# vainaviv/hulk-keypoints

Measured on NVIDIA B200. Metric: heatmap_inference_images_per_sec, higher is better.
Workload: dtype bf16

## Files before the change

### hulk_keypoints_b200/csrc/conv_tc.cu

```cuda
#include <cuda.h>

#include "hk_common.cuh"
#include "hk_ptx.cuh"

namespace hk {

constexpr int TC_BLOCK_M = 128;
constexpr int TC_BLOCK_K = 64;
constexpr int TC_UMMA_K = 16;
constexpr int TC_BOX_H = 4, TC_BOX_W = 16;
constexpr int TC_BOX_PIX = TC_BOX_H * TC_BOX_W;
constexpr int TC_BOX_BYTES = TC_BOX_PIX * TC_BLOCK_K * 2;
constexpr int TC_A_BYTES = TC_BLOCK_M * TC_BLOCK_K * 2;
constexpr int TC_THREADS = 256;
constexpr int TC_EPI_WARP0 = 4;

struct ConvTcArgs {
  const float* scale;
  const float* bias;
  const __nv_bfloat16* residual;
  __nv_bfloat16* y;
  int B, Ho, Wo, Cout;
  int Cin, kh, kw, stride, pad, dil, relu;
  int tiles_x, tiles_per_img, num_boxes;
  int num_m_tiles, num_n_tiles, cblocks;
};

template <int BLOCK_N>
struct TcCfg {
  static constexpr int B_BYTES = BLOCK_N * TC_BLOCK_K * 2;
  static constexpr int STAGE_BYTES = TC_A_BYTES + B_BYTES;
  static constexpr int STAGES = (192 * 1024) / STAGE_BYTES > 8 ? 8 : (192 * 1024) / STAGE_BYTES;
  static constexpr int TMEM_COLS = 2 * BLOCK_N;
  static constexpr int SMEM_BYTES = STAGES * STAGE_BYTES + 1024  + 256 ;
};

__device__ __forceinline__ void tc_decode_box(const ConvTcArgs& a, int box, int& b, int& y0, int& x0) {
  if (box < a.num_boxes) {
    b = box / a.tiles_per_img;
    const int r = box - b * a.tiles_per_img;
    const int ty = r / a.tiles_x;
    y0 = ty * TC_BOX_H;
    x0 = (r - ty * a.tiles_x) * TC_BOX_W;
  } else {
    b = a.B;
    y0 = 0;
    x0 = 0;
  }
}

template <int BLOCK_N>
__global__ void __launch_bounds__(TC_THREADS, 1)
conv_tc_kernel(const __grid_constant__ CUtensorMap map_x, const __grid_constant__ CUtensorMap map_w, const ConvTcArgs a) {
  using Cfg = TcCfg<BLOCK_N>;
  constexpr int STAGES = Cfg::STAGES;
  extern __shared__ uint8_t smem_raw[];
  uint8_t* smem = smem_raw + ((1024u - (ptx::smem_u32(smem_raw) & 1023u)) & 1023u);
  uint64_t* full_bar = reinterpret_cast<uint64_t*>(smem + STAGES * Cfg::STAGE_BYTES);
  uint64_t* empty_bar = full_bar + STAGES;
  uint64_t* tmem_full_bar = empty_bar + STAGES;
  uint64_t* tmem_empty_bar = tmem_full_bar + 2;
  uint32_t* tmem_ptr_smem = reinterpret_cast<uint32_t*>(tmem_empty_bar + 2);

  const int warp = __shfl_sync(0xffffffffu, threadIdx.x >> 5, 0), lane = threadIdx.x & 31;
  const int total_tiles = a.num_m_tiles * a.num_n_tiles;
  const int num_kb = a.kh * a.kw * a.cblocks;

  if (warp == 0 && lane == 0) {
    ptx::prefetch_tensormap(&map_x);
    ptx::prefetch_tensormap(&map_w);
  }
  if (warp == 1 && lane == 0) {
    for (int i = 0; i < STAGES; ++i) {
      ptx::mbar_init(&full_bar[i], 1);
      ptx::mbar_init(&empty_bar[i], 1);
    }
    for (int i = 0; i < 2; ++i) {
      ptx::mbar_init(&tmem_full_bar[i], 1);
      ptx::mbar_init(&tmem_empty_bar[i], 128);
    }
    ptx::fence_mbar_init();
  }
  if (warp == 2) {
    ptx::tmem_alloc(tmem_ptr_smem, Cfg::TMEM_COLS);
    ptx::tmem_relinquish();
  }
  ptx::tc_fence_before();
  __syncthreads();
  ptx::tc_fence_after();
  const uint32_t tmem_base = *tmem_ptr_smem;

  if (warp == 0) {
    {
      uint32_t stage = 0, phase = 0;
      for (int tile = blockIdx.x; tile < total_tiles; tile += gridDim.x) {
        const int m_tile = tile / a.num_n_tiles, n_tile = tile - m_tile * a.num_n_tiles;
        int b0, y0, x0, b1, y1, x1;
        tc_decode_box(a, 2 * m_tile, b0, y0, x0);
        tc_decode_box(a, 2 * m_tile + 1, b1, y1, x1);
        for (int r = 0; r < a.kh; ++r) {
          for (int s = 0; s < a.kw; ++s) {
            const int dy = r * a.dil - a.pad, dx = s * a.dil - a.pad;
            const int kbase = (r * a.kw + s) * a.Cin;
            for (int cb = 0; cb < a.cblocks; ++cb) {
              ptx::mbar_wait(&empty_bar[stage], phase ^ 1, 1);
              if (ptx::elect_one_sync()) {
                uint8_t* sa = smem + stage * Cfg::STAGE_BYTES;
                ptx::mbar_arrive_expect_tx(&full_bar[stage], Cfg::STAGE_BYTES);
                ptx::tma_load_4d(sa, &map_x, &full_bar[stage], cb * TC_BLOCK_K, x0 * a.stride + dx, y0 * a.stride + dy, b0);
                ptx::tma_load_4d(sa + TC_BOX_BYTES, &map_x, &full_bar[stage], cb * TC_BLOCK_K, x1 * a.stride + dx,
                                 y1 * a.stride + dy, b1);
                ptx::tma_load_2d(sa + TC_A_BYTES, &map_w, &full_bar[stage], kbase + cb * TC_BLOCK_K, n_tile * BLOCK_N);
              }
              __syncwarp();
              if (++stage == STAGES) { stage = 0; phase ^= 1; }
            }
          }
        }
      }
    }
  } else if (warp == 1) {
    {
      constexpr uint32_t idesc = ptx::make_idesc_bf16_f32(TC_BLOCK_M, BLOCK_N);
      uint32_t stage = 0, phase = 0, it = 0;
      for (int tile = blockIdx.x; tile < total_tiles; tile += gridDim.x, ++it) {
        const uint32_t acc = it & 1, acc_phase = (it >> 1) & 1;
        ptx::mbar_wait(&tmem_empty_bar[acc], acc_phase ^ 1, 2);
        ptx::tc_fence_after();
        const uint32_t d_tmem = tmem_base + acc * BLOCK_N;
        for (int kb = 0; kb < num_kb; ++kb) {
          ptx::mbar_wait(&full_bar[stage], phase, 3);
          ptx::tc_fence_after();
          const uint32_t sa = ptx::smem_u32(smem + stage * Cfg::STAGE_BYTES);
          const uint64_t adesc = ptx::make_smem_desc_sw128(sa);
          const uint64_t bdesc = ptx::make_smem_desc_sw128(sa + TC_A_BYTES);
          if (ptx::elect_one_sync()) {
#pragma unroll
            for (int k = 0; k < TC_BLOCK_K / TC_UMMA_K; ++k) {
              ptx::umma_bf16(d_tmem, adesc + 2 * k, bdesc + 2 * k, idesc, (kb | k) != 0 ? 1u : 0u);
            }
            ptx::umma_commit(&empty_bar[stage]);
            if (kb == num_kb - 1) ptx::umma_commit(&tmem_full_bar[acc]);
          }
          __syncwarp();
          if (++stage == STAGES) { stage = 0; phase ^= 1; }
        }
      }
    }
  } else if (warp >= TC_EPI_WARP0) {
    const int q = warp & 3;
    const int row = q * 32 + lane;
    const int py = (row & 63) >> 4, px = row & 15;
    uint32_t it = 0;
    for (int tile = blockIdx.x; tile < total_tiles; tile += gridDim.x, ++it) {
      const uint32_t acc = it & 1, acc_phase = (it >> 1) & 1;
      const int m_tile = tile / a.num_n_tiles, n_tile = tile - m_tile * a.num_n_tiles;
      int b, y0, x0;
      tc_decode_box(a, 2 * m_tile + (row >> 6), b, y0, x0);
      const int oy = y0 + py, ox = x0 + px;
      const bool valid = (b < a.B) && (oy < a.Ho) && (ox < a.Wo);
      const size_t off = valid ? (((size_t)b * a.Ho + oy) * a.Wo + ox) * a.Cout + (size_t)n_tile * BLOCK_N : 0;
      const float* scale = a.scale + n_tile * BLOCK_N;
      const float* bias = a.bias + n_tile * BLOCK_N;

      ptx::mbar_wait(&tmem_full_bar[acc], acc_phase, 4);
      ptx::tc_fence_after();
      const uint32_t taddr = tmem_base + (static_cast<uint32_t>(q * 32) << 16) + acc * BLOCK_N;
#pragma unroll 1
      for (int c0 = 0; c0 < BLOCK_N; c0 += 32) {
        uint32_t r[32];
        ptx::tmem_ld_32x32(taddr + c0, r);
        ptx::tmem_ld_wait();
        if (valid) {
#pragma unroll
          for (int g = 0; g < 4; ++g) {
            const int c = c0 + g * 8;
            const float4 s0 = __ldg(reinterpret_cast<const float4*>(scale + c));
            const float4 s1 = __ldg(reinterpret_cast<const float4*>(scale + c + 4));
            const float4 t0 = __ldg(reinterpret_cast<const float4*>(bias + c));
            const float4 t1 = __ldg(reinterpret_cast<const float4*>(bias + c + 4));
            float v[8];
            v[0] = fmaf(__uint_as_float(r[g * 8 + 0]), s0.x, t0.x);
            v[1] = fmaf(__uint_as_float(r[g * 8 + 1]), s0.y, t0.y);
            v[2] = fmaf(__uint_as_float(r[g * 8 + 2]), s0.z, t0.z);
            v[3] = fmaf(__uint_as_float(r[g * 8 + 3]), s0.w, t0.w);
            v[4] = fmaf(__uint_as_float(r[g * 8 + 4]), s1.x, t1.x);
            v[5] = fmaf(__uint_as_float(r[g * 8 + 5]), s1.y, t1.y);
            v[6] = fmaf(__uint_as_float(r[g * 8 + 6]), s1.z, t1.z);
            v[7] = fmaf(__uint_as_float(r[g * 8 + 7]), s1.w, t1.w);
            if (a.residual) {
              const uint4 rq = __ldg(reinterpret_cast<const uint4*>(a.residual + off + c));
              float lo, hi;
              unpack_bf16x2(rq.x, lo, hi); v[0] += lo; v[1] += hi;
              unpack_bf16x2(rq.y, lo, hi); v[2] += lo; v[3] += hi;
              unpack_bf16x2(rq.z, lo, hi); v[4] += lo; v[5] += hi;
              unpack_bf16x2(rq.w, lo, hi); v[6] += lo; v[7] += hi;
            }
            if (a.relu) {
#pragma unroll
              for (int j = 0; j < 8; ++j) v[j] = fmaxf(v[j], 0.f);
            }
            *reinterpret_cast<uint4*>(a.y + off + c) =
                make_uint4(pack_bf16x2(v[0], v[1]), pack_bf16x2(v[2], v[3]), pack_bf16x2(v[4], v[5]), pack_bf16x2(v[6], v[7]));
          }
        }
      }
      ptx::tc_fence_before();
      ptx::mbar_arrive(&tmem_empty_bar[acc]);
    }
  }

  ptx::tc_fence_before();
  __syncthreads();
  if (warp == 2) {
    ptx::tc_fence_after();
    ptx::tmem_dealloc(tmem_base, Cfg::TMEM_COLS);
  }
}

typedef CUresult (*EncodeTiledFn)(CUtensorMap*, CUtensorMapDataType, cuuint32_t, void*, const cuuint64_t*, const cuuint64_t*,
                                  const cuuint32_t*, const cuuint32_t*, CUtensorMapInterleave, CUtensorMapSwizzle,
                                  CUtensorMapL2promotion, CUtensorMapFloatOOBfill);

EncodeTiledFn get_encode_fn() {
  static EncodeTiledFn fn = nullptr;
  static bool tried = false;
  if (!tried) {
    tried = true;
    void* p = nullptr;
    cudaDriverEntryPointQueryResult q;
    if (cudaGetDriverEntryPoint("cuTensorMapEncodeTiled", &p, cudaEnableDefault, &q) == cudaSuccess &&
        q == cudaDriverEntryPointSuccess)
      fn = reinterpret_cast<EncodeTiledFn>(p);
  }
  return fn;
}

template <int BLOCK_N>
static int launch_tc(const CUtensorMap& mx, const CUtensorMap& mw, const ConvTcArgs& a, cudaStream_t s) {
  using Cfg = TcCfg<BLOCK_N>;
  static bool attr_set = false;
  int dev = 0;
  cudaGetDevice(&dev);
  static int attr_dev_mask = 0;
  if (!attr_set || !(attr_dev_mask & (1 << dev))) {
    cudaError_t e = cudaFuncSetAttribute(conv_tc_kernel<BLOCK_N>, cudaFuncAttributeMaxDynamicSharedMemorySize, Cfg::SMEM_BYTES);
    if (e != cudaSuccess) return fail(HK_ERR_CUDA, "conv(tcgen05): smem attribute (%d B): %s", Cfg::SMEM_BYTES, cudaGetErrorString(e));
    attr_set = true;
    attr_dev_mask |= (1 << dev);
  }
  const int total = a.num_m_tiles * a.num_n_tiles;
  int grid = sm_count();
  if (grid > total) grid = total;
  conv_tc_kernel<BLOCK_N><<<grid, TC_THREADS, Cfg::SMEM_BYTES, s>>>(mx, mw, a);
  return check_launch("conv_tc_kernel");
}

bool conv_tc2_applicable(const HkConvDesc& d);
int conv_tc2_launch(const HkConvDesc& d, const void* x, const void* w, const float* scale, const float* bias,
                    const void* residual, void* y, void* bn_acc, cudaStream_t s);
bool conv_tc2h_applicable(const HkConvDesc& d);
int conv_tc2h_launch(const HkConvDesc& d, const void* x, const void* w, const float* scale, const float* bias,
                     const void* residual, void* y, void* bn_acc, cudaStream_t s);
bool conv_tc_c64_applicable(const HkConvDesc& d);
int conv_tc_c64_launch(const HkConvDesc& d, const void* x, const void* w, const float* scale, const float* bias,
                       const void* residual, void* y, void* bn_acc, cudaStream_t s);

int conv_tc_launch(const HkConvDesc& d, const void* x, const void* w, const float* scale, const float* bias,
                   const void* residual, void* y, cudaStream_t s, void* bn_acc = nullptr, bool* stats_done = nullptr) {
  if (stats_done) *stats_done = false;
  HK_REQUIRE(d.in_dtype == HK_BF16 && d.out_dtype == HK_BF16 && !d.in_is_nchw, "conv(tcgen05): needs NHWC bf16 in and out");
  HK_REQUIRE(d.in_c % TC_BLOCK_K == 0, "conv(tcgen05): in_c=%d must be a multiple of 64", d.in_c);
  HK_REQUIRE(d.out_c % 64 == 0, "conv(tcgen05): out_c=%d must be a multiple of 64", d.out_c);
  HK_REQUIRE(d.stride == 1 || d.stride == 2, "conv(tcgen05): stride must be 1 or 2");
  HK_REQUIRE((reinterpret_cast<uintptr_t>(x) & 15) == 0 && (reinterpret_cast<uintptr_t>(w) & 15) == 0 &&
                 (reinterpret_cast<uintptr_t>(y) & 15) == 0 && (reinterpret_cast<uintptr_t>(residual) & 15) == 0,
             "conv(tcgen05): buffers must be 16-byte aligned");
  EncodeTiledFn encode = get_encode_fn();
  if (!encode) return fail(HK_ERR_CUDA, "conv(tcgen05): cuTensorMapEncodeTiled entry point not available");

  const bool specialised = d.algo != HK_CONV_TCGEN05_1CTA;
  if (stats_done) *stats_done = bn_acc && specialised && (conv_tc_c64_applicable(d) || conv_tc2_applicable(d));
  if (specialised && conv_tc_c64_applicable(d)) return conv_tc_c64_launch(d, x, w, scale, bias, residual, y, bn_acc, s);
  if (specialised && conv_tc2_applicable(d) && conv_tc2h_applicable(d)) return conv_tc2h_launch(d, x, w, scale, bias, residual, y, bn_acc, s);
  if (specialised && conv_tc2_applicable(d)) return conv_tc2_launch(d, x, w, scale, bias, residual, y, bn_acc, s);

  const int block_n = d.out_c % 256 == 0 ? 256 : (d.out_c % 128 == 0 ? 128 : 64);
  const int ktot = d.kh * d.kw * d.in_c;

  CUtensorMap mx, mw;
  {
    const cuuint64_t dims[4] = {(cuuint64_t)d.in_c, (cuuint64_t)d.in_w, (cuuint64_t)d.in_h, (cuuint64_t)d.batch};
    const cuuint64_t strides[3] = {(cuuint64_t)d.in_c * 2, (cuuint64_t)d.in_w * d.in_c * 2, (cuuint64_t)d.in_h * d.in_w * d.in_c * 2};
    const cuuint32_t box[4] = {(cuuint32_t)TC_BLOCK_K, (cuuint32_t)(TC_BOX_W * d.stride), (cuuint32_t)(TC_BOX_H * d.stride), 1};
    const cuuint32_t estr[4] = {1, (cuuint32_t)d.stride, (cuuint32_t)d.stride, 1};
    CUresult r = encode(&mx, CU_TENSOR_MAP_DATA_TYPE_BFLOAT16, 4, const_cast<void*>(x), dims, strides, box, estr,
                        CU_TENSOR_MAP_INTERLEAVE_NONE, CU_TENSOR_MAP_SWIZZLE_128B, CU_TENSOR_MAP_L2_PROMOTION_L2_128B,
                        CU_TENSOR_MAP_FLOAT_OOB_FILL_NONE);
    if (r != CUDA_SUCCESS) return fail(HK_ERR_CUDA, "conv(tcgen05): cuTensorMapEncodeTiled(activations) failed with CUresult %d", (int)r);
  }
  {
    const cuuint64_t dims[2] = {(cuuint64_t)ktot, (cuuint64_t)d.out_c};
    const cuuint64_t strides[1] = {(cuuint64_t)ktot * 2};
    const cuuint32_t box[2] = {(cuuint32_t)TC_BLOCK_K, (cuuint32_t)block_n};
    const cuuint32_t estr[2] = {1, 1};
    CUresult r = encode(&mw, CU_TENSOR_MAP_DATA_TYPE_BFLOAT16, 2, const_cast<void*>(w), dims, strides, box, estr,
                        CU_TENSOR_MAP_INTERLEAVE_NONE, CU_TENSOR_MAP_SWIZZLE_128B, CU_TENSOR_MAP_L2_PROMOTION_L2_256B,
                        CU_TENSOR_MAP_FLOAT_OOB_FILL_NONE);
    if (r != CUDA_SUCCESS) return fail(HK_ERR_CUDA, "conv(tcgen05): cuTensorMapEncodeTiled(weights) failed with CUresult %d", (int)r);
  }

  ConvTcArgs a;
  a.scale = scale; a.bias = bias;
  a.residual = static_cast<const __nv_bfloat16*>(residual);
  a.y = static_cast<__nv_bfloat16*>(y);
  a.B = d.batch; a.Ho = d.out_h; a.Wo = d.out_w; a.Cout = d.out_c;
  a.Cin = d.in_c; a.kh = d.kh; a.kw = d.kw; a.stride = d.stride; a.pad = d.pad; a.dil = d.dil; a.relu = d.relu;
  a.tiles_x = ceil_div(d.out_w, TC_BOX_W);
  a.tiles_per_img = a.tiles_x * ceil_div(d.out_h, TC_BOX_H);
  const long long boxes = (long long)a.tiles_per_img * d.batch;
  HK_REQUIRE(boxes < 0x3fffffffLL, "conv(tcgen05): too many tiles");
  a.num_boxes = (int)boxes;
  a.num_m_tiles = (a.num_boxes + 1) / 2;
  a.num_n_tiles = d.out_c / block_n;
  a.cblocks = d.in_c / TC_BLOCK_K;
  switch (block_n) {
    case 256: return launch_tc<256>(mx, mw, a, s);
    case 128: return launch_tc<128>(mx, mw, a, s);
    default: return launch_tc<64>(mx, mw, a, s);
  }
}

int conv_ffma_launch(const HkConvDesc& d, const void* x, const void* w, const float* scale, const float* bias,
                     const void* residual, void* y, cudaStream_t s);

}

extern "C" int hk_conv_bn_act_fwd(const HkConvDesc* desc, const void* x, const void* w_packed, const float* scale,
                                  const float* bias, const void* residual_or_null, void* y, void* stream) {
  using namespace hk;
  HK_REQUIRE(desc && x && w_packed && scale && bias && y, "hk_conv_bn_act_fwd: null pointer");
  const HkConvDesc& d = *desc;
  HK_REQUIRE(d.batch > 0 && d.in_h > 0 && d.in_w > 0 && d.in_c > 0 && d.out_c > 0 && d.kh > 0 && d.kw > 0 && d.stride > 0 &&
                 d.dil > 0 && d.pad >= 0,
             "hk_conv_bn_act_fwd: bad descriptor");
  const int eh = d.dil * (d.kh - 1) + 1, ew = d.dil * (d.kw - 1) + 1;
  HK_REQUIRE(d.in_h + 2 * d.pad >= eh && d.in_w + 2 * d.pad >= ew, "hk_conv_bn_act_fwd: kernel larger than padded input");
  HK_REQUIRE(d.out_h == (d.in_h + 2 * d.pad - eh) / d.stride + 1 && d.out_w == (d.in_w + 2 * d.pad - ew) / d.stride + 1,
             "hk_conv_bn_act_fwd: out_h/out_w (%d,%d) inconsistent with the descriptor", d.out_h, d.out_w);
  if (d.algo == HK_CONV_TCGEN05 || d.algo == HK_CONV_TCGEN05_1CTA) return conv_tc_launch(d, x, w_packed, scale, bias, residual_or_null, y, as_stream(stream));
  if (d.algo == HK_CONV_FFMA) return conv_ffma_launch(d, x, w_packed, scale, bias, residual_or_null, y, as_stream(stream));
  return fail(HK_ERR_BAD_ARG, "hk_conv_bn_act_fwd: unknown algo %d", d.algo);
}

extern "C" int hk_bn_stats_acc(const void* y, long long P, int C, void* acc, void* stream);
extern "C" int hk_conv_bn_stats_fwd(const HkConvDesc* desc, const void* x, const void* w_packed, const float* scale, const float* bias,
                                    void* y, void* acc, void* stream) {
  using namespace hk;
  HK_REQUIRE(desc && x && w_packed && scale && bias && y && acc, "hk_conv_bn_stats_fwd: null pointer");
  const HkConvDesc& d = *desc;
  HK_REQUIRE(d.algo == HK_CONV_TCGEN05 && d.in_dtype == HK_BF16 && d.out_dtype == HK_BF16 && !d.in_is_nchw && !d.relu,
             "hk_conv_bn_stats_fwd: tcgen05 path only (NHWC bf16 in and out, no ReLU: BatchNorm sees the raw conv output)");
  HK_REQUIRE(d.batch > 0 && d.in_h > 0 && d.in_w > 0 && d.in_c > 0 && d.out_c > 0 && d.kh > 0 && d.kw > 0 && d.stride > 0 && d.dil > 0 && d.pad >= 0,
             "hk_conv_bn_stats_fwd: bad descriptor");
  const int eh = d.dil * (d.kh - 1) + 1, ew = d.dil * (d.kw - 1) + 1;
  HK_REQUIRE(d.out_h == (d.in_h + 2 * d.pad - eh) / d.stride + 1 && d.out_w == (d.in_w + 2 * d.pad - ew) / d.stride + 1,
             "hk_conv_bn_stats_fwd: out_h/out_w (%d,%d) inconsistent with the descriptor", d.out_h, d.out_w);
  HK_REQUIRE((reinterpret_cast<uintptr_t>(acc) & 31) == 0, "hk_conv_bn_stats_fwd: accumulators must be 32-byte aligned");
  bool done = false;
  int rc = conv_tc_launch(d, x, w_packed, scale, bias, nullptr, y, as_stream(stream), acc, &done);
  if (rc || done) return rc;
  return hk_bn_stats_acc(y, (long long)d.batch * d.out_h * d.out_w, d.out_c, acc, stream);
}
```

### hulk_keypoints_b200/csrc/conv_tc2h.cu

```cuda
#include <cuda.h>
#include <stdlib.h>

#include "hk_common.cuh"
#include "hk_bn_acc.cuh"
#include "hk_ptx.cuh"
#include "hk_ptx2.cuh"

namespace hk {

constexpr int TH_TILE_H = 8, TH_TILE_W = 16;
constexpr int TH_ROW_BYTES = TH_TILE_W * 128;
constexpr int TH_THREADS = 384;
constexpr int TH_EPI_THREADS = 256;
constexpr int TH_STAGING_BYTES = 3 * 128 * 128;
constexpr int TH_MAX_A = 4, TH_MAX_B = 8;

struct ConvTc2hArgs {
  const float* scale;
  const float* bias;
  const __nv_bfloat16* residual;
  int B, Ho, Wo, Cout, Cin, pad, dil, relu;
  int tiles_x, tiles_per_img, num_patches;
  int strip_first, num_strips, strips_per_img, strip_y0;
  int num_m_tiles, num_n_tiles, cblocks;
  int a_slot_bytes, a_bytes_full, a_bytes_strip, a_slots, b_slots;
  BnAcc* bn_acc;
};

__device__ __forceinline__ void th_decode_patch(const ConvTc2hArgs& a, int patch, int& b, int& y0, int& x0) {
  if (patch < a.num_patches) {
    b = patch / a.tiles_per_img;
    const int r = patch - b * a.tiles_per_img;
    const int ty = r / a.tiles_x;
    y0 = ty * TH_TILE_H;
    x0 = (r - ty * a.tiles_x) * TH_TILE_W;
  } else if (patch >= a.strip_first && patch < a.strip_first + a.num_strips) {
    const int q = patch - a.strip_first;
    b = q / a.strips_per_img;
    y0 = a.strip_y0;
    x0 = (q - b * a.strips_per_img) * (2 * TH_TILE_W);
  } else {
    b = a.B;
    y0 = 0;
    x0 = 0;
  }
}

template <int BLOCK_N, bool STATS>
__global__ void __cluster_dims__(2, 1, 1) __launch_bounds__(TH_THREADS, 1)
conv_tc2h_kernel(const __grid_constant__ CUtensorMap map_x, const __grid_constant__ CUtensorMap map_w,
                 const __grid_constant__ CUtensorMap map_y, const __grid_constant__ CUtensorMap map_res,
                 const __grid_constant__ CUtensorMap map_xs, const __grid_constant__ CUtensorMap map_ys,
                 const __grid_constant__ CUtensorMap map_ress, const ConvTc2hArgs a) {
  constexpr int HALF_N = BLOCK_N / 2;
  constexpr int B_BYTES = HALF_N * 128;
  extern __shared__ uint8_t smem_raw[];
  uint8_t* smem = smem_raw + ((1024u - (ptx::smem_u32(smem_raw) & 1023u)) & 1023u);
  const int NA = a.a_slots, NB = a.b_slots;
  uint8_t* sA = smem;
  uint8_t* sB = sA + NA * a.a_slot_bytes;
  uint8_t* staging = sB + NB * B_BYTES;
  uint64_t* a_full = reinterpret_cast<uint64_t*>(staging + TH_STAGING_BYTES);
  uint64_t* a_empty = a_full + TH_MAX_A;
  uint64_t* b_full = a_empty + TH_MAX_A;
  uint64_t* b_empty = b_full + TH_MAX_B;
  uint64_t* tmem_full_bar = b_empty + TH_MAX_B;
  uint64_t* tmem_empty_bar = tmem_full_bar + 2;
  uint64_t* res_bar = tmem_empty_bar + 2;
  uint32_t* tmem_ptr_smem = reinterpret_cast<uint32_t*>(res_bar + 3);

  const int warp = __shfl_sync(0xffffffffu, threadIdx.x >> 5, 0), lane = threadIdx.x & 31;
  const uint32_t rank = ptx::cluster_ctarank();
  const bool leader = rank == 0;
  const int cluster_id = blockIdx.x >> 1, num_clusters = gridDim.x >> 1;
  const int total_tiles = a.num_m_tiles * a.num_n_tiles;

  ptx::griddep_launch_dependents();
  ptx::cluster_sync_all();
  if (warp == 0 && lane == 0) {
    ptx::prefetch_tensormap(&map_x);
    ptx::prefetch_tensormap(&map_w);
    ptx::prefetch_tensormap(&map_y);
    if (a.residual) ptx::prefetch_tensormap(&map_res);
    if (a.num_strips > 0) {
      ptx::prefetch_tensormap(&map_xs);
      ptx::prefetch_tensormap(&map_ys);
      if (a.residual) ptx::prefetch_tensormap(&map_ress);
    }
  }
  if (warp == 1 && lane == 0) {
    for (int i = 0; i < TH_MAX_A; ++i) {
      ptx::mbar_init(&a_full[i], 2);
      ptx::mbar_init(&a_empty[i], 1);
    }
    for (int i = 0; i < TH_MAX_B; ++i) {
      ptx::mbar_init(&b_full[i], 2);
      ptx::mbar_init(&b_empty[i], 1);
    }
    for (int i = 0; i < 2; ++i) {
      ptx::mbar_init(&tmem_full_bar[i], 1);
      ptx::mbar_init(&tmem_empty_bar[i], 2 * TH_EPI_THREADS);
    }
    for (int i = 0; i < 3; ++i) ptx::mbar_init(&res_bar[i], 1);
    ptx::fence_mbar_init();
  }
  if (warp == 2) {
    ptx::tmem_alloc2(tmem_ptr_smem, 2 * BLOCK_N);
    ptx::tmem_relinquish2();
  }
  ptx::tc_fence_before();
  ptx::cluster_sync_all();
  ptx::tc_fence_after();
  const uint32_t tmem_base = *tmem_ptr_smem;

  if (warp == 0) {
    ptx::griddep_wait();
    uint32_t as = 0, aph = 0, bs = 0, bph = 0;
    for (int tile = cluster_id; tile < total_tiles; tile += num_clusters) {
      const int m_tile = tile / a.num_n_tiles, n_tile = tile - m_tile * a.num_n_tiles;
      int b, y0, x0;
      th_decode_patch(a, 2 * m_tile + (int)rank, b, y0, x0);
      const bool strip = 2 * m_tile >= a.strip_first;
      const CUtensorMap* mxp = strip ? &map_xs : &map_x;
      const uint32_t a_tx = 2u * (uint32_t)(strip ? a.a_bytes_strip : a.a_bytes_full);
      const int n_row0 = n_tile * BLOCK_N + (int)rank * HALF_N;
      for (int s = 0; s < 3; ++s) {
        for (int cb = 0; cb < a.cblocks; ++cb) {
          ptx::mbar_wait(&a_empty[as], aph ^ 1, 51);
          if (ptx::elect_one_sync()) {
            ptx::tma2_load_4d(sA + as * a.a_slot_bytes, mxp, &a_full[as], cb * 64, x0 + (s - 1) * a.dil, y0 - a.dil, b);
            if (leader) ptx::mbar_arrive_expect_tx(&a_full[as], a_tx);
            else ptx::mbar_arrive_remote(&a_full[as], 0);
          }
          __syncwarp();
          if (++as == (uint32_t)NA) { as = 0; aph ^= 1; }
          for (int r = 0; r < 3; ++r) {
            ptx::mbar_wait(&b_empty[bs], bph ^ 1, 52);
            if (ptx::elect_one_sync()) {
              ptx::tma2_load_2d(sB + bs * B_BYTES, &map_w, &b_full[bs], (r * 3 + s) * a.Cin + cb * 64, n_row0);
              if (leader) ptx::mbar_arrive_expect_tx(&b_full[bs], 2 * B_BYTES);
              else ptx::mbar_arrive_remote(&b_full[bs], 0);
            }
            __syncwarp();
            if (++bs == (uint32_t)NB) { bs = 0; bph ^= 1; }
          }
        }
      }
    }
  } else if (warp == 1) {
    if (leader) {
      constexpr uint32_t idesc = ptx::make_idesc_bf16_f32(256, BLOCK_N);
      uint32_t as = 0, aph = 0, bs = 0, bph = 0, it = 0;
      for (int tile = cluster_id; tile < total_tiles; tile += num_clusters, ++it) {
        const uint32_t acc = it & 1, acc_phase = (it >> 1) & 1;
        const bool strip = 2 * (tile / a.num_n_tiles) >= a.strip_first;
        const uint32_t tap_bytes = (uint32_t)a.dil * (strip ? 2 * TH_ROW_BYTES : TH_ROW_BYTES);
        ptx::mbar_wait(&tmem_empty_bar[acc], acc_phase ^ 1, 53);
        ptx::tc_fence_after();
        const uint32_t d_tmem = tmem_base + acc * BLOCK_N;
        const int groups = 3 * a.cblocks;
        for (int g = 0; g < groups; ++g) {
          ptx::mbar_wait(&a_full[as], aph, 54);
          const uint32_t a_base = ptx::smem_u32(sA + as * a.a_slot_bytes);
          for (int r = 0; r < 3; ++r) {
            ptx::mbar_wait(&b_full[bs], bph, 55);
            ptx::tc_fence_after();
            if (ptx::elect_one_sync()) {
              const uint64_t adesc = ptx::make_smem_desc_sw128(a_base + r * tap_bytes);
              const uint64_t bdesc = ptx::make_smem_desc_sw128(ptx::smem_u32(sB + bs * B_BYTES));
#pragma unroll
              for (int k = 0; k < 4; ++k) ptx::umma2_bf16(d_tmem, adesc + 2 * k, bdesc + 2 * k, idesc, (g | r | k) != 0 ? 1u : 0u);
              ptx::umma2_commit_mc(&b_empty[bs]);
              if (r == 2) {
                ptx::umma2_commit_mc(&a_empty[as]);
                if (g == groups - 1) ptx::umma2_commit_mc(&tmem_full_bar[acc]);
              }
            }
            __syncwarp();
            if (++bs == (uint32_t)NB) { bs = 0; bph ^= 1; }
          }
          if (++as == (uint32_t)NA) { as = 0; aph ^= 1; }
        }
      }
      if (it >= 1) { const uint32_t j = it - 1; ptx::mbar_wait(&tmem_empty_bar[j & 1], (j >> 1) & 1, 56); }
      if (it >= 2) { const uint32_t j = it - 2; ptx::mbar_wait(&tmem_empty_bar[j & 1], (j >> 1) & 1, 57); }
    }
  } else if (warp >= 4) {
    const int q = warp & 3, half = (warp - 4) >> 2;
    const int row = q * 32 + lane;
    const bool elected = (warp == 4 && lane == 0);
    const int sw = row & 7;
    constexpr int CHUNKS = BLOCK_N / 64;
    const bool has_res = a.residual != nullptr;
    const int et = (int)threadIdx.x - 128;
    EpiStats stats;
    if (STATS) epi_stats_init(stats, reinterpret_cast<float*>(reinterpret_cast<uint8_t*>(a_full) + 512), a.Cout, et);
    ptx::griddep_wait();
    uint32_t it = 0, chunk_ctr = 0;
    for (int tile = cluster_id; tile < total_tiles; tile += num_clusters, ++it) {
      const uint32_t acc = it & 1, acc_phase = (it >> 1) & 1;
      const int m_tile = tile / a.num_n_tiles, n_tile = tile - m_tile * a.num_n_tiles;
      int b, y0, x0;
      th_decode_patch(a, 2 * m_tile + (int)rank, b, y0, x0);
      const bool strip = 2 * m_tile >= a.strip_first;
      const CUtensorMap* myp = strip ? &map_ys : &map_y;
      const CUtensorMap* mrp = strip ? &map_ress : &map_res;
      const int n0 = n_tile * BLOCK_N;
      const float* scale = a.scale + n0;
      const float* bias = a.bias + n0;
      int nvalid = 0;
      if (STATS) {
        const int rg = et >> 5;
        const int yy = y0 + (strip ? rg >> 1 : rg), xx = x0 + (strip ? (rg & 1) * 16 : 0);
        if (b < a.B && yy < a.Ho) nvalid = min(16, max(0, a.Wo - xx));
      }
      auto issue_residual = [&](int chunk, uint32_t ctr) {
        const uint32_t bsel = ctr % 3;
        ptx::mbar_arrive_expect_tx(&res_bar[bsel], 16384);
        ptx::tma_load_4d(staging + bsel * 16384, mrp, &res_bar[bsel], n0 + chunk * 64, x0, y0, b);
      };
      if (elected) {
        ptx::bulk_wait_group_read1();
        if (has_res) issue_residual(0, chunk_ctr);
      }
      ptx::mbar_wait(&tmem_full_bar[acc], acc_phase, 58);
      ptx::tc_fence_after();
      const uint32_t taddr = tmem_base + (static_cast<uint32_t>(q * 32) << 16) + acc * BLOCK_N;
#pragma unroll 1
      for (int chunk = 0; chunk < CHUNKS; ++chunk, ++chunk_ctr) {
        const uint32_t bsel = chunk_ctr % 3;
        uint8_t* my_row = staging + bsel * 16384 + row * 128;
        if (elected) {
          ptx::bulk_wait_group_read1();
          if (has_res && chunk + 1 < CHUNKS) issue_residual(chunk + 1, chunk_ctr + 1);
        }
        ptx::named_bar_sync(1, TH_EPI_THREADS);
        if (STATS) epi_stats_reduce_prev(stats, et);
        uint32_t r0[32];
        ptx::tmem_ld_32x32(taddr + chunk * 64 + half * 32, r0);
        ptx::tmem_ld_wait();
        if (chunk == CHUNKS - 1) {
          ptx::tc_fence_before();
          ptx::mbar_arrive_remote(&tmem_empty_bar[acc], 0);
        }
        if (has_res) ptx::mbar_wait(&res_bar[bsel], (chunk_ctr / 3) & 1, 59);
#pragma unroll
        for (int gg = 0; gg < 4; ++gg) {
          const int g = half * 4 + gg;
          const int c = chunk * 64 + g * 8;
          const float4 s0 = __ldg(reinterpret_cast<const float4*>(scale + c));
          const float4 s1 = __ldg(reinterpret_cast<const float4*>(scale + c + 4));
          const float4 t0 = __ldg(reinterpret_cast<const float4*>(bias + c));
          const float4 t1 = __ldg(reinterpret_cast<const float4*>(bias + c + 4));
          const float sc[8] = {s0.x, s0.y, s0.z, s0.w, s1.x, s1.y, s1.z, s1.w};
          const float bi[8] = {t0.x, t0.y, t0.z, t0.w, t1.x, t1.y, t1.z, t1.w};
          float v[8];
#pragma unroll
          for (int j = 0; j < 8; ++j) v[j] = fmaf(__uint_as_float(r0[gg * 8 + j]), sc[j], bi[j]);
          uint4* slot = reinterpret_cast<uint4*>(my_row + (((g ^ sw) & 7) << 4));
          if (has_res) {
            const uint4 rr = *slot;
            float lo, hi;
            unpack_bf16x2(rr.x, lo, hi); v[0] += lo; v[1] += hi;
            unpack_bf16x2(rr.y, lo, hi); v[2] += lo; v[3] += hi;
            unpack_bf16x2(rr.z, lo, hi); v[4] += lo; v[5] += hi;
            unpack_bf16x2(rr.w, lo, hi); v[6] += lo; v[7] += hi;
          }
          if (a.relu) {
#pragma unroll
            for (int j = 0; j < 8; ++j) v[j] = fmaxf(v[j], 0.f);
          }
          *slot = make_uint4(pack_bf16x2(v[0], v[1]), pack_bf16x2(v[2], v[3]), pack_bf16x2(v[4], v[5]), pack_bf16x2(v[6], v[7]));
        }
        ptx::fence_proxy_async_smem();
        ptx::named_bar_sync(1, TH_EPI_THREADS);
        if (elected) {
          ptx::tma_store_4d(myp, staging + bsel * 16384, n0 + chunk * 64, x0, y0, b);
          ptx::bulk_commit_group();
        }
        if (STATS) epi_stats_chunk(stats, staging + bsel * 16384, et, nvalid, n0 + chunk * 64);
      }
    }
    if (STATS) epi_stats_flush(stats, et, a.Cout, a.bn_acc, [] { ptx::named_bar_sync(1, TH_EPI_THREADS); });
    if (elected) ptx::bulk_wait_group0();
  }

  ptx::tc_fence_before();
  ptx::cluster_sync_all();
  if (warp == 2) {
    ptx::tc_fence_after();
    ptx::tmem_dealloc2(tmem_base, 2 * BLOCK_N);
  }
}

typedef CUresult (*EncodeTiledFn)(CUtensorMap*, CUtensorMapDataType, cuuint32_t, void*, const cuuint64_t*, const cuuint64_t*,
                                  const cuuint32_t*, const cuuint32_t*, CUtensorMapInterleave, CUtensorMapSwizzle,
                                  CUtensorMapL2promotion, CUtensorMapFloatOOBfill);
EncodeTiledFn get_encode_fn();

bool conv_tc2h_applicable(const HkConvDesc& d) {
  const char* env = getenv("HK_CONV_HALO");
  if (env && env[0] == '0') return false;
  if (!(d.kh == 3 && d.kw == 3 && d.stride == 1 && d.pad == d.dil && d.out_c % 128 == 0 && d.in_c % 64 == 0)) return false;
  if (d.dil != 1 && d.dil != 2 && d.dil != 4) return false;
  if (env && env[0] == '1') return true;
  return d.dil <= 2;
}

template <int BLOCK_N, bool STATS>
static int launch_tc2h(const CUtensorMap& mx, const CUtensorMap& mw, const CUtensorMap& my, const CUtensorMap& mres,
                       const CUtensorMap& mxs, const CUtensorMap& mys, const CUtensorMap& mress, ConvTc2hArgs& a, cudaStream_t s) {
  constexpr int B_BYTES = (BLOCK_N / 2) * 128;
  const int stats_bytes = STATS ? epi_stats_smem_bytes(a.Cout) : 0;
  const int budget = 227 * 1024 - 1024 - TH_STAGING_BYTES - 512 - stats_bytes;
  int na = 3, nb = (budget - na * a.a_slot_bytes) / B_BYTES;
  if (nb > TH_MAX_B) {
    nb = TH_MAX_B;
    if ((budget - nb * B_BYTES) / a.a_slot_bytes >= 4) na = 4;
  }
  if (nb < 3) return fail(HK_ERR_BAD_ARG, "conv(tcgen05,halo): shared memory budget too small");
  a.a_slots = na;
  a.b_slots = nb;
  const int smem = 1024 + na * a.a_slot_bytes + nb * B_BYTES + TH_STAGING_BYTES + 512 + stats_bytes;
  static int attr_smem[16] = {0};
  int dev = 0;
  cudaGetDevice(&dev);
  if (dev < 16 && attr_smem[dev] < smem) {
    cudaError_t e = cudaFuncSetAttribute(conv_tc2h_kernel<BLOCK_N, STATS>, cudaFuncAttributeMaxDynamicSharedMemorySize, smem);
    if (e != cudaSuccess) return fail(HK_ERR_CUDA, "conv(tcgen05,halo): smem attribute (%d B): %s", smem, cudaGetErrorString(e));
    attr_smem[dev] = smem;
  }
  const int total = a.num_m_tiles * a.num_n_tiles;
  int clusters = sm_count() / 2;
  if (clusters > total) clusters = total;
  cudaError_t le = launch_pdl(conv_tc2h_kernel<BLOCK_N, STATS>, dim3(2 * clusters), dim3(TH_THREADS), (size_t)smem, s, mx, mw, my, mres, mxs, mys,
                              mress, a);
  if (le != cudaSuccess) return fail(HK_ERR_CUDA, "conv_tc2h_kernel: %s", cudaGetErrorString(le));
  return check_launch("conv_tc2h_kernel");
}

int conv_tc2h_launch(const HkConvDesc& d, const void* x, const void* w, const float* scale, const float* bias, const void* residual,
                     void* y, void* bn_acc, cudaStream_t s) {
  EncodeTiledFn encode = get_encode_fn();
  if (!encode) return fail(HK_ERR_CUDA, "conv(tcgen05,halo): cuTensorMapEncodeTiled entry point not available");
  const char* strips_env = getenv("HK_CONV_STRIPS");
  const int rem_rows = d.out_h % TH_TILE_H;
  const bool use_strips = !(strips_env && strips_env[0] == '0') && rem_rows >= 1 && rem_rows <= 4 && d.out_h > TH_TILE_H && d.dil <= 2;
  const int tiles_x = ceil_div(d.out_w, TH_TILE_W);
  const int tiles_y = use_strips ? d.out_h / TH_TILE_H : ceil_div(d.out_h, TH_TILE_H);
  const int strips_per_img = use_strips ? ceil_div(d.out_w, 2 * TH_TILE_W) : 0;
  const long long full_all = (long long)tiles_x * tiles_y * d.batch;
  const long long strip_first_ll = (full_all + 1) / 2 * 2;
  const long long strips_all = (long long)strips_per_img * d.batch;
  const long long patches_all = use_strips ? strip_first_ll + strips_all : full_all;
  const int block_n = pick_block_n_pair(d.out_c, (patches_all + 1) / 2);
  const int ktot = 9 * d.in_c;
  const int box_rows = TH_TILE_H + 2 * d.dil;
  const int strip_box_rows = TH_TILE_H / 2 + 2 * d.dil;
  CUtensorMap mx, mw, my, mres;
  {
    const cuuint64_t dims[4] = {(cuuint64_t)d.in_c, (cuuint64_t)d.in_w, (cuuint64_t)d.in_h, (cuuint64_t)d.batch};
    const cuuint64_t strides[3] = {(cuuint64_t)d.in_c * 2, (cuuint64_t)d.in_w * d.in_c * 2, (cuuint64_t)d.in_h * d.in_w * d.in_c * 2};
    const cuuint32_t box[4] = {64, (cuuint32_t)TH_TILE_W, (cuuint32_t)box_rows, 1};
    const cuuint32_t estr[4] = {1, 1, 1, 1};
    CUresult r = encode(&mx, CU_TENSOR_MAP_DATA_TYPE_BFLOAT16, 4, const_cast<void*>(x), dims, strides, box, estr,
                        CU_TENSOR_MAP_INTERLEAVE_NONE, CU_TENSOR_MAP_SWIZZLE_128B, CU_TENSOR_MAP_L2_PROMOTION_L2_128B,
                        CU_TENSOR_MAP_FLOAT_OOB_FILL_NONE);
    if (r != CUDA_SUCCESS) return fail(HK_ERR_CUDA, "conv(tcgen05,halo): cuTensorMapEncodeTiled(activations) failed: %d", (int)r);
  }
  {
    const cuuint64_t dims[2] = {(cuuint64_t)ktot, (cuuint64_t)d.out_c};
    const cuuint64_t strides[1] = {(cuuint64_t)ktot * 2};
    const cuuint32_t box[2] = {64, (cuuint32_t)(block_n / 2)};
    const cuuint32_t estr[2] = {1, 1};
    CUresult r = encode(&mw, CU_TENSOR_MAP_DATA_TYPE_BFLOAT16, 2, const_cast<void*>(w), dims, strides, box, estr,
                        CU_TENSOR_MAP_INTERLEAVE_NONE, CU_TENSOR_MAP_SWIZZLE_128B, CU_TENSOR_MAP_L2_PROMOTION_L2_256B,
                        CU_TENSOR_MAP_FLOAT_OOB_FILL_NONE);
    if (r != CUDA_SUCCESS) return fail(HK_ERR_CUDA, "conv(tcgen05,halo): cuTensorMapEncodeTiled(weights) failed: %d", (int)r);
  }
  {
    const cuuint64_t dims[4] = {(cuuint64_t)d.out_c, (cuuint64_t)d.out_w, (cuuint64_t)d.out_h, (cuuint64_t)d.batch};
    const cuuint64_t strides[3] = {(cuuint64_t)d.out_c * 2, (cuuint64_t)d.out_w * d.out_c * 2, (cuuint64_t)d.out_h * d.out_w * d.out_c * 2};
    const cuuint32_t box[4] = {64, (cuuint32_t)TH_TILE_W, (cuuint32_t)TH_TILE_H, 1};
    const cuuint32_t estr[4] = {1, 1, 1, 1};
    CUresult r = encode(&my, CU_TENSOR_MAP_DATA_TYPE_BFLOAT16, 4, y, dims, strides, box, estr, CU_TENSOR_MAP_INTERLEAVE_NONE,
                        CU_TENSOR_MAP_SWIZZLE_128B, CU_TENSOR_MAP_L2_PROMOTION_L2_128B, CU_TENSOR_MAP_FLOAT_OOB_FILL_NONE);
    if (r != CUDA_SUCCESS) return fail(HK_ERR_CUDA, "conv(tcgen05,halo): cuTensorMapEncodeTiled(output) failed: %d", (int)r);
    mres = my;
    if (residual) {
      r = encode(&mres, CU_TENSOR_MAP_DATA_TYPE_BFLOAT16, 4, const_cast<void*>(residual), dims, strides, box, estr,
                 CU_TENSOR_MAP_INTERLEAVE_NONE, CU_TENSOR_MAP_SWIZZLE_128B, CU_TENSOR_MAP_L2_PROMOTION_L2_128B,
                 CU_TENSOR_MAP_FLOAT_OOB_FILL_NONE);
      if (r != CUDA_SUCCESS) return fail(HK_ERR_CUDA, "conv(tcgen05,halo): cuTensorMapEncodeTiled(residual) failed: %d", (int)r);
    }
  }
  CUtensorMap mxs = mx, mys = my, mress = mres;
  if (use_strips) {
    const cuuint32_t estr[4] = {1, 1, 1, 1};
    {
      const cuuint64_t dims[4] = {(cuuint64_t)d.in_c, (cuuint64_t)d.in_w, (cuuint64_t)d.in_h, (cuuint64_t)d.batch};
      const cuuint64_t strides[3] = {(cuuint64_t)d.in_c * 2, (cuuint64_t)d.in_w * d.in_c * 2, (cuuint64_t)d.in_h * d.in_w * d.in_c * 2};
      const cuuint32_t box[4] = {64, (cuuint32_t)(2 * TH_TILE_W), (cuuint32_t)strip_box_rows, 1};
      CUresult r = encode(&mxs, CU_TENSOR_MAP_DATA_TYPE_BFLOAT16, 4, const_cast<void*>(x), dims, strides, box, estr,
                          CU_TENSOR_MAP_INTERLEAVE_NONE, CU_TENSOR_MAP_SWIZZLE_128B, CU_TENSOR_MAP_L2_PROMOTION_L2_128B,
                          CU_TENSOR_MAP_FLOAT_OOB_FILL_NONE);
      if (r != CUDA_SUCCESS) return fail(HK_ERR_CUDA, "conv(tcgen05,halo): cuTensorMapEncodeTiled(strip activations) failed: %d", (int)r);
    }
    const cuuint64_t dims[4] = {(cuuint64_t)d.out_c, (cuuint64_t)d.out_w, (cuuint64_t)d.out_h, (cuuint64_t)d.batch};
    const cuuint64_t strides[3] = {(cuuint64_t)d.out_c * 2, (cuuint64_t)d.out_w * d.out_c * 2, (cuuint64_t)d.out_h * d.out_w * d.out_c * 2};
    const cuuint32_t box[4] = {64, (cuuint32_t)(2 * TH_TILE_W), (cuuint32_t)(TH_TILE_H / 2), 1};
    CUresult r = encode(&mys, CU_TENSOR_MAP_DATA_TYPE_BFLOAT16, 4, y, dims, strides, box, estr, CU_TENSOR_MAP_INTERLEAVE_NONE,
                        CU_TENSOR_MAP_SWIZZLE_128B, CU_TENSOR_MAP_L2_PROMOTION_L2_128B, CU_TENSOR_MAP_FLOAT_OOB_FILL_NONE);
    if (r != CUDA_SUCCESS) return fail(HK_ERR_CUDA, "conv(tcgen05,halo): cuTensorMapEncodeTiled(strip output) failed: %d", (int)r);
    mress = mys;
    if (residual) {
      r = encode(&mress, CU_TENSOR_MAP_DATA_TYPE_BFLOAT16, 4, const_cast<void*>(residual), dims, strides, box, estr,
                 CU_TENSOR_MAP_INTERLEAVE_NONE, CU_TENSOR_MAP_SWIZZLE_128B, CU_TENSOR_MAP_L2_PROMOTION_L2_128B,
                 CU_TENSOR_MAP_FLOAT_OOB_FILL_NONE);
      if (r != CUDA_SUCCESS) return fail(HK_ERR_CUDA, "conv(tcgen05,halo): cuTensorMapEncodeTiled(strip residual) failed: %d", (int)r);
    }
  }
  ConvTc2hArgs a;
  a.scale = scale; a.bias = bias;
  a.residual = static_cast<const __nv_bfloat16*>(residual);
  a.B = d.batch; a.Ho = d.out_h; a.Wo = d.out_w; a.Cout = d.out_c; a.Cin = d.in_c; a.pad = d.pad; a.dil = d.dil; a.relu = d.relu;
  a.tiles_x = tiles_x;
  a.tiles_per_img = tiles_x * tiles_y;
  HK_REQUIRE(patches_all < 0x3fffffffLL, "conv(tcgen05,halo): too many tiles");
  a.num_patches = (int)full_all;
  a.strip_first = use_strips ? (int)strip_first_ll : 0x7fffffff;
  a.num_strips = (int)strips_all;
  a.strips_per_img = strips_per_img > 0 ? strips_per_img : 1;
  a.strip_y0 = tiles_y * TH_TILE_H;
  a.num_m_tiles = (int)((patches_all + 1) / 2);
  a.num_n_tiles = d.out_c / block_n;
  a.cblocks = d.in_c / 64;
  a.a_bytes_full = box_rows * TH_ROW_BYTES;
  a.a_bytes_strip = strip_box_rows * 2 * TH_ROW_BYTES;
  a.a_slot_bytes = use_strips && a.a_bytes_strip > a.a_bytes_full ? a.a_bytes_strip : a.a_bytes_full;
  a.bn_acc = static_cast<BnAcc*>(bn_acc);
  if (bn_acc) return block_n == 256 ? launch_tc2h<256, true>(mx, mw, my, mres, mxs, mys, mress, a, s) : launch_tc2h<128, true>(mx, mw, my, mres, mxs, mys, mress, a, s);
  return block_n == 256 ? launch_tc2h<256, false>(mx, mw, my, mres, mxs, mys, mress, a, s) : launch_tc2h<128, false>(mx, mw, my, mres, mxs, mys, mress, a, s);
}

}
```

Measured before the change: 6321.

## Route Cin=Cout=64 convs to paired halo kernel with resident weights

For 64-channel 3x3 convs without residual or BN statistics, dispatch now goes to the 2-CTA halo-tile kernel instead of the single-CTA c64 kernel, using a new BLOCK_N=64 instantiation. In that mode all nine weight taps are loaded into shared memory once per CTA and kept resident, which removes the per-tap B-operand pipeline waits and commits. The freed shared memory is spent on more A-operand slots (up to 6). This adds a new template instantiation and an env-var escape hatch. The gain depends on how many 64-channel layers the network has and how well a 256x64 pair UMMA uses the tensor cores.

```diff
diff --git a/hulk_keypoints_b200/csrc/conv_tc.cu b/hulk_keypoints_b200/csrc/conv_tc.cu
--- a/hulk_keypoints_b200/csrc/conv_tc.cu
+++ b/hulk_keypoints_b200/csrc/conv_tc.cu
@@ -281,7 +281,11 @@
 
   const bool specialised = d.algo != HK_CONV_TCGEN05_1CTA;
   if (stats_done) *stats_done = bn_acc && specialised && (conv_tc_c64_applicable(d) || conv_tc2_applicable(d));
-  if (specialised && conv_tc_c64_applicable(d)) return conv_tc_c64_launch(d, x, w, scale, bias, residual, y, bn_acc, s);
+  if (specialised && conv_tc_c64_applicable(d)) {
+    const char* pair_env = getenv("HK_C64_PAIR");
+    if (!bn_acc && !residual && !(pair_env && pair_env[0] == '0')) return conv_tc2h_launch(d, x, w, scale, bias, nullptr, y, nullptr, s);
+    return conv_tc_c64_launch(d, x, w, scale, bias, residual, y, bn_acc, s);
+  }
   if (specialised && conv_tc2_applicable(d) && conv_tc2h_applicable(d)) return conv_tc2h_launch(d, x, w, scale, bias, residual, y, bn_acc, s);
   if (specialised && conv_tc2_applicable(d)) return conv_tc2_launch(d, x, w, scale, bias, residual, y, bn_acc, s);
 
diff --git a/hulk_keypoints_b200/csrc/conv_tc2h.cu b/hulk_keypoints_b200/csrc/conv_tc2h.cu
--- a/hulk_keypoints_b200/csrc/conv_tc2h.cu
+++ b/hulk_keypoints_b200/csrc/conv_tc2h.cu
@@ -13,7 +13,7 @@
 constexpr int TH_THREADS = 384;
 constexpr int TH_EPI_THREADS = 256;
 constexpr int TH_STAGING_BYTES = 3 * 128 * 128;
-constexpr int TH_MAX_A = 4, TH_MAX_B = 8;
+constexpr int TH_MAX_A = 6, TH_MAX_B = 8;
 
 struct ConvTc2hArgs {
   const float* scale;
@@ -54,6 +54,7 @@
                  const __grid_constant__ CUtensorMap map_ress, const ConvTc2hArgs a) {
   constexpr int HALF_N = BLOCK_N / 2;
   constexpr int B_BYTES = HALF_N * 128;
+  constexpr bool RES_W = BLOCK_N == 64;
   extern __shared__ uint8_t smem_raw[];
   uint8_t* smem = smem_raw + ((1024u - (ptx::smem_u32(smem_raw) & 1023u)) & 1023u);
   const int NA = a.a_slots, NB = a.b_slots;
@@ -116,6 +117,14 @@
   if (warp == 0) {
     ptx::griddep_wait();
     uint32_t as = 0, aph = 0, bs = 0, bph = 0;
+    if (RES_W) {
+      if (ptx::elect_one_sync()) {
+        for (int t = 0; t < 9; ++t) ptx::tma2_load_2d(sB + t * B_BYTES, &map_w, &b_full[0], t * 64, (int)rank * HALF_N);
+        if (leader) ptx::mbar_arrive_expect_tx(&b_full[0], 2 * 9 * B_BYTES);
+        else ptx::mbar_arrive_remote(&b_full[0], 0);
+      }
+      __syncwarp();
+    }
     for (int tile = cluster_id; tile < total_tiles; tile += num_clusters) {
       const int m_tile = tile / a.num_n_tiles, n_tile = tile - m_tile * a.num_n_tiles;
       int b, y0, x0;
@@ -134,7 +143,7 @@
           }
           __syncwarp();
           if (++as == (uint32_t)NA) { as = 0; aph ^= 1; }
-          for (int r = 0; r < 3; ++r) {
+          for (int r = 0; r < 3 && !RES_W; ++r) {
             ptx::mbar_wait(&b_empty[bs], bph ^ 1, 52);
             if (ptx::elect_one_sync()) {
               ptx::tma2_load_2d(sB + bs * B_BYTES, &map_w, &b_full[bs], (r * 3 + s) * a.Cin + cb * 64, n_row0);
@@ -151,6 +160,7 @@
     if (leader) {
       constexpr uint32_t idesc = ptx::make_idesc_bf16_f32(256, BLOCK_N);
       uint32_t as = 0, aph = 0, bs = 0, bph = 0, it = 0;
+      if (RES_W) ptx::mbar_wait(&b_full[0], 0, 55);
       for (int tile = cluster_id; tile < total_tiles; tile += num_clusters, ++it) {
         const uint32_t acc = it & 1, acc_phase = (it >> 1) & 1;
         const bool strip = 2 * (tile / a.num_n_tiles) >= a.strip_first;
@@ -163,21 +173,21 @@
           ptx::mbar_wait(&a_full[as], aph, 54);
           const uint32_t a_base = ptx::smem_u32(sA + as * a.a_slot_bytes);
           for (int r = 0; r < 3; ++r) {
-            ptx::mbar_wait(&b_full[bs], bph, 55);
+            if (!RES_W) ptx::mbar_wait(&b_full[bs], bph, 55);
             ptx::tc_fence_after();
             if (ptx::elect_one_sync()) {
               const uint64_t adesc = ptx::make_smem_desc_sw128(a_base + r * tap_bytes);
-              const uint64_t bdesc = ptx::make_smem_desc_sw128(ptx::smem_u32(sB + bs * B_BYTES));
+              const uint64_t bdesc = ptx::make_smem_desc_sw128(ptx::smem_u32(sB + (RES_W ? r * 3 + g : (int)bs) * B_BYTES));
 #pragma unroll
               for (int k = 0; k < 4; ++k) ptx::umma2_bf16(d_tmem, adesc + 2 * k, bdesc + 2 * k, idesc, (g | r | k) != 0 ? 1u : 0u);
-              ptx::umma2_commit_mc(&b_empty[bs]);
+              if (!RES_W) ptx::umma2_commit_mc(&b_empty[bs]);
               if (r == 2) {
                 ptx::umma2_commit_mc(&a_empty[as]);
                 if (g == groups - 1) ptx::umma2_commit_mc(&tmem_full_bar[acc]);
               }
             }
             __syncwarp();
-            if (++bs == (uint32_t)NB) { bs = 0; bph ^= 1; }
+            if (!RES_W && ++bs == (uint32_t)NB) { bs = 0; bph ^= 1; }
           }
           if (++as == (uint32_t)NA) { as = 0; aph ^= 1; }
         }
@@ -314,7 +324,12 @@
   const int stats_bytes = STATS ? epi_stats_smem_bytes(a.Cout) : 0;
   const int budget = 227 * 1024 - 1024 - TH_STAGING_BYTES - 512 - stats_bytes;
   int na = 3, nb = (budget - na * a.a_slot_bytes) / B_BYTES;
-  if (nb > TH_MAX_B) {
+  if (BLOCK_N == 64) {
+    nb = 9;
+    na = (budget - nb * B_BYTES) / a.a_slot_bytes;
+    if (na > TH_MAX_A) na = TH_MAX_A;
+    if (na < 3) return fail(HK_ERR_BAD_ARG, "conv(tcgen05,halo): shared memory budget too small");
+  } else if (nb > TH_MAX_B) {
     nb = TH_MAX_B;
     if ((budget - nb * B_BYTES) / a.a_slot_bytes >= 4) na = 4;
   }
@@ -353,7 +368,7 @@
   const long long strip_first_ll = (full_all + 1) / 2 * 2;
   const long long strips_all = (long long)strips_per_img * d.batch;
   const long long patches_all = use_strips ? strip_first_ll + strips_all : full_all;
-  const int block_n = pick_block_n_pair(d.out_c, (patches_all + 1) / 2);
+  const int block_n = d.out_c == 64 ? 64 : pick_block_n_pair(d.out_c, (patches_all + 1) / 2);
   const int ktot = 9 * d.in_c;
   const int box_rows = TH_TILE_H + 2 * d.dil;
   const int strip_box_rows = TH_TILE_H / 2 + 2 * d.dil;
@@ -439,6 +454,10 @@
   a.a_bytes_strip = strip_box_rows * 2 * TH_ROW_BYTES;
   a.a_slot_bytes = use_strips && a.a_bytes_strip > a.a_bytes_full ? a.a_bytes_strip : a.a_bytes_full;
   a.bn_acc = static_cast<BnAcc*>(bn_acc);
+  if (block_n == 64) {
+    HK_REQUIRE(d.in_c == 64 && !bn_acc, "conv(tcgen05,halo): N=64 tiles need Cin = 64 and no epilogue statistics");
+    return launch_tc2h<64, false>(mx, mw, my, mres, mxs, mys, mress, a, s);
+  }
   if (bn_acc) return block_n == 256 ? launch_tc2h<256, true>(mx, mw, my, mres, mxs, mys, mress, a, s) : launch_tc2h<128, true>(mx, mw, my, mres, mxs, mys, mress, a, s);
   return block_n == 256 ? launch_tc2h<256, false>(mx, mw, my, mres, mxs, mys, mress, a, s) : launch_tc2h<128, false>(mx, mw, my, mres, mxs, mys, mress, a, s);
 }
```

Result: no change. 6332, median of 6 (+0.2%).
